# Horizon1026/Feature_Detector

Hardware: AMD Instinct MI355X
Metric: Mpix/s corner-response+NMS, 640x480 gray batch, 1/2/4/8 MI355X (higher is better)
Workload: dtype u8->i32/f32; 1 GPU; harris response+NMS + grid NMS (greedy min-distance select), 640x480 gray, batch 1/GPU (BASELINE configs[1]); detector=harris, rows=480, cols=640, global_batch=1, need=200, min_feature_distance=20, parallelism=frame-sharded x1 (no collective), graph=True

## Files before the change

### feature_detector_amd/csrc/fd_device.h

```cpp
#pragma once

#include <hip/hip_runtime.h>
#include <stdint.h>

namespace fdk {

constexpr int kWave = 64;

__device__ __forceinline__ int lane_id() { return threadIdx.x & 63; }

__device__ __forceinline__ uint32_t from_left(uint32_t v) {
    return static_cast<uint32_t>(__builtin_amdgcn_mov_dpp(static_cast<int>(v), 0x138, 0xF, 0xF, true));
}
__device__ __forceinline__ uint32_t from_right(uint32_t v) {
    return static_cast<uint32_t>(__builtin_amdgcn_mov_dpp(static_cast<int>(v), 0x130, 0xF, 0xF, true));
}
__device__ __forceinline__ float from_left_f(float v) { return __uint_as_float(from_left(__float_as_uint(v))); }
__device__ __forceinline__ float from_right_f(float v) { return __uint_as_float(from_right(__float_as_uint(v))); }

__device__ __forceinline__ __amdgpu_buffer_rsrc_t make_rsrc(const void *base, uint32_t bytes) {
    return __builtin_amdgcn_make_buffer_rsrc(const_cast<void *>(base), 0, static_cast<int>(bytes), 0x00020000);
}
__device__ __forceinline__ uint32_t buf_load_u32(__amdgpu_buffer_rsrc_t r, int32_t byte_off) {
    return static_cast<uint32_t>(__builtin_amdgcn_raw_buffer_load_b32(r, byte_off, 0, 0));
}
__device__ __forceinline__ uint32_t buf_load_u8(__amdgpu_buffer_rsrc_t r, int32_t byte_off) {
    return static_cast<uint32_t>(__builtin_amdgcn_raw_buffer_load_b8(r, byte_off, 0, 0));
}

__device__ __forceinline__ int win_byte(uint32_t L, uint32_t M, uint32_t R, int j) {
    const uint32_t w = j < 0 ? L : (j < 4 ? M : R);
    const int sh = 8 * (j < 0 ? j + 4 : (j < 4 ? j : j - 4));
    return static_cast<int>((w >> sh) & 0xFFu);
}

__device__ __forceinline__ float max3f(float a, float b, float c) {
    float r;
    asm("v_max3_f32 %0, %1, %2, %3" : "=v"(r) : "v"(a), "v"(b), "v"(c));
    return r;
}

__device__ __forceinline__ uint32_t add3u(uint32_t a, uint32_t b, uint32_t c) {
    uint32_t r;
    asm("v_add3_u32 %0, %1, %2, %3" : "=v"(r) : "v"(a), "v"(b), "v"(c));
    return r;
}

__device__ __forceinline__ uint32_t wave_incl_add(uint32_t x) {
    x += static_cast<uint32_t>(__builtin_amdgcn_update_dpp(0, static_cast<int>(x), 0x111, 0xF, 0xF, false));
    x += static_cast<uint32_t>(__builtin_amdgcn_update_dpp(0, static_cast<int>(x), 0x112, 0xF, 0xF, false));
    x += static_cast<uint32_t>(__builtin_amdgcn_update_dpp(0, static_cast<int>(x), 0x114, 0xF, 0xF, false));
    x += static_cast<uint32_t>(__builtin_amdgcn_update_dpp(0, static_cast<int>(x), 0x118, 0xF, 0xF, false));
    x += static_cast<uint32_t>(__builtin_amdgcn_update_dpp(0, static_cast<int>(x), 0x142, 0xA, 0xF, false));
    x += static_cast<uint32_t>(__builtin_amdgcn_update_dpp(0, static_cast<int>(x), 0x143, 0xC, 0xF, false));
    return x;
}
__device__ __forceinline__ uint32_t wave_max_u32(uint32_t x) {
    x = max(x, static_cast<uint32_t>(__builtin_amdgcn_update_dpp(0, static_cast<int>(x), 0x111, 0xF, 0xF, false)));
    x = max(x, static_cast<uint32_t>(__builtin_amdgcn_update_dpp(0, static_cast<int>(x), 0x112, 0xF, 0xF, false)));
    x = max(x, static_cast<uint32_t>(__builtin_amdgcn_update_dpp(0, static_cast<int>(x), 0x114, 0xF, 0xF, false)));
    x = max(x, static_cast<uint32_t>(__builtin_amdgcn_update_dpp(0, static_cast<int>(x), 0x118, 0xF, 0xF, false)));
    x = max(x, static_cast<uint32_t>(__builtin_amdgcn_update_dpp(0, static_cast<int>(x), 0x142, 0xA, 0xF, false)));
    x = max(x, static_cast<uint32_t>(__builtin_amdgcn_update_dpp(0, static_cast<int>(x), 0x143, 0xC, 0xF, false)));
    return static_cast<uint32_t>(__builtin_amdgcn_readlane(static_cast<int>(x), 63));
}
__device__ __forceinline__ uint32_t wave_min_u32(uint32_t x) {
    x = min(x, static_cast<uint32_t>(__builtin_amdgcn_update_dpp(-1, static_cast<int>(x), 0x111, 0xF, 0xF, false)));
    x = min(x, static_cast<uint32_t>(__builtin_amdgcn_update_dpp(-1, static_cast<int>(x), 0x112, 0xF, 0xF, false)));
    x = min(x, static_cast<uint32_t>(__builtin_amdgcn_update_dpp(-1, static_cast<int>(x), 0x114, 0xF, 0xF, false)));
    x = min(x, static_cast<uint32_t>(__builtin_amdgcn_update_dpp(-1, static_cast<int>(x), 0x118, 0xF, 0xF, false)));
    x = min(x, static_cast<uint32_t>(__builtin_amdgcn_update_dpp(-1, static_cast<int>(x), 0x142, 0xA, 0xF, false)));
    x = min(x, static_cast<uint32_t>(__builtin_amdgcn_update_dpp(-1, static_cast<int>(x), 0x143, 0xC, 0xF, false)));
    return static_cast<uint32_t>(__builtin_amdgcn_readlane(static_cast<int>(x), 63));
}
__device__ __forceinline__ uint32_t wave_total_add(uint32_t x) {
    return static_cast<uint32_t>(__builtin_amdgcn_readlane(static_cast<int>(wave_incl_add(x)), 63));
}
__device__ __forceinline__ uint32_t wave_suffix_add(uint32_t x) {
    const uint32_t p = wave_incl_add(x);
    const uint32_t tot = static_cast<uint32_t>(__builtin_amdgcn_readlane(static_cast<int>(p), 63));
    return tot - p + x;
}

__device__ __forceinline__ int opaque(int x) {
    asm volatile("" : "+v"(x));
    return x;
}

template <class T>
using lds_t = __attribute__((address_space(3))) T;
template <class T>
__device__ __forceinline__ lds_t<T> *to_lds(T *p) { return (lds_t<T> *)(p); }
template <class T>
__device__ __forceinline__ T *from_lds(lds_t<T> *p) { return (T *)(p); }

__device__ __forceinline__ uint64_t ballot(bool p) { return __ballot(p); }
__device__ __forceinline__ int popc64(uint64_t m) { return __popcll(m); }
__device__ __forceinline__ uint64_t lanes_below() {
    const int l = lane_id();
    return l == 0 ? 0ull : (~0ull >> (64 - l));
}

__device__ __forceinline__ int mbcnt64(uint64_t m, int acc) {
    const uint32_t lo = __builtin_amdgcn_mbcnt_lo(static_cast<uint32_t>(m), static_cast<uint32_t>(acc));
    return static_cast<int>(__builtin_amdgcn_mbcnt_hi(static_cast<uint32_t>(m >> 32), lo));
}

template <int NT>
__device__ __forceinline__ uint32_t wg_excl_add(uint32_t v, uint32_t *wsum, uint32_t &tot) {
    constexpr int kWaves = NT / kWave;
    const int lane = lane_id(), w = threadIdx.x / kWave;
    const uint32_t incl = wave_incl_add(v);
    if (lane == kWave - 1) wsum[w] = incl;
    __syncthreads();
    const uint32_t ws = lane < kWaves ? wsum[lane] : 0u;
    const uint32_t wincl = wave_incl_add(ws);
    const uint32_t wbase = static_cast<uint32_t>(__shfl(static_cast<int>(wincl - ws), w));
    tot = static_cast<uint32_t>(__builtin_amdgcn_readlane(static_cast<int>(wincl), kWaves - 1));
    __syncthreads();
    return wbase + incl - v;
}

__device__ __forceinline__ uint32_t float_key(float f) {
    const uint32_t u = __float_as_uint(f);
    return (u & 0x80000000u) ? ~u : (u | 0x80000000u);
}

typedef float f2 __attribute__((ext_vector_type(2)));

__device__ __forceinline__ f2 sqrt_rn_rsq2(f2 x) {
    const f2 xt = x + 0x1p-110f;
    const f2 y = {__builtin_amdgcn_rsqf(xt.x), __builtin_amdgcn_rsqf(xt.y)};
    const f2 s0 = x * y;
    const f2 e = __builtin_elementwise_fma(-s0, s0, x);
    const f2 h = y * 0.5f;
    return __builtin_elementwise_fma(e, h, s0);
}

}
```

### feature_detector_amd/csrc/fd_emit.h

```cpp
#pragma once

#include "fd_device.h"
#include "fd_kernels.h"

namespace fdk {

__device__ __forceinline__ uint32_t sel_key32(float resp, uint32_t key_base, int key_lz) {
    return (float_key(resp) - key_base) << key_lz;
}
__device__ __forceinline__ uint64_t sel_key64(float resp, uint32_t idx, uint32_t key_base, int key_lz, int tie_desc) {
    return (static_cast<uint64_t>(sel_key32(resp, key_base, key_lz)) << 32) | static_cast<uint64_t>(tie_desc ? idx : ~idx);
}
__device__ __forceinline__ uint32_t level0_bin(float resp, uint32_t key_base, int key_lz) {
    return sel_key32(resp, key_base, key_lz) >> 20;
}
__device__ __forceinline__ uint32_t level0_floor_key(uint32_t bin, uint32_t key_base, int key_lz) {
    return key_base + ((bin << 20) >> key_lz);
}

struct ListFrame {
    float *resp;
    uint32_t *idx;
    int64_t cap;
};
__device__ __forceinline__ ListFrame list_frame(const CandList &l, int f) {
    return {l.resp + static_cast<int64_t>(f) * l.cap, l.idx + static_cast<int64_t>(f) * l.cap, l.cap};
}

constexpr int kPixWg = 256;
constexpr int kHistPer = kHistBins / (4 * kPixWg);
__device__ __forceinline__ void hist_clear(uint32_t *h) {
    uint4 *h4 = reinterpret_cast<uint4 *>(h);
#pragma unroll
    for (int k = 0; k < kHistPer; ++k) h4[threadIdx.x + k * kPixWg] = make_uint4(0u, 0u, 0u, 0u);
    __syncthreads();
}
__device__ __forceinline__ void hist_flush(const uint32_t *h, uint32_t *g) {
    __syncthreads();
    constexpr int kPer = kHistBins / kPixWg;
    uint32_t v[kPer];
#pragma unroll
    for (int k = 0; k < kPer; ++k) v[k] = h[threadIdx.x + k * kPixWg];
#pragma unroll
    for (int k = 0; k < kPer; ++k)
        if (v[k]) atomicAdd(&g[threadIdx.x + k * kPixWg], v[k]);
}

__device__ __forceinline__ void wave_append(const CandList &l, int f, const float *sr, const uint32_t *si, int n,
                                            uint32_t *hist) {
    uint32_t base = 0;
    if (lane_id() == 0) base = atomicAdd(&l.count[f], static_cast<uint32_t>(n));
    base = __builtin_amdgcn_readfirstlane(base);
    const ListFrame d = list_frame(l, f);
    for (int i = lane_id(); i < n; i += kWave) {
        const float r = sr[i];
        if (hist) atomicAdd(&hist[level0_bin(r, l.key_base, l.key_lz)], 1u);
        const int64_t pos = static_cast<int64_t>(base) + i;
        if (pos < d.cap) {
            d.resp[pos] = r;
            d.idx[pos] = si[i];
        }
    }
}

template <class Src>
__device__ __forceinline__ void seg_list_flush(Src &src, const PointsArgs &a, int f, int g, bool active, uint32_t *hist,
                                               const uint32_t *ovf, uint32_t (&wtot)[4], uint32_t &wg_base) {
    const int tid = threadIdx.x, lane = lane_id(), wv = tid >> 6;
    if (!active) src.n = 0;
    const uint32_t wn = src.wave_total();
    if (lane == 0) wtot[wv] = wn;
    __syncthreads();
    if (*ovf) {
        if (active) src.flush(a, f);
        hist_flush(hist, a.list.hist0 + static_cast<int64_t>(f) * kHistBins);
        return;
    }
    uint32_t seg_base_early = 0;
    const uint32_t seg_total = wtot[0] + wtot[1] + wtot[2] + wtot[3];
    if (tid == 0 && seg_total) seg_base_early = atomicAdd(&a.list.count[f], seg_total);
    const uint32_t kb = a.list.key_base;
    const int lz = a.list.key_lz;
    if (!src.counted()) src.visit([&](float r, uint32_t) { atomicAdd(&hist[level0_bin(r, kb, lz)], 1u); });
    hist_flush(hist, a.list.hist0 + static_cast<int64_t>(f) * kHistBins);
    __syncthreads();
    constexpr int kPer = kHistBins / kPixWg;
    uint32_t v[kPer], sum = 0;
#pragma unroll
    for (int k = 0; k < kPer; ++k) sum += (v[k] = hist[kHistBins - 1 - (tid * kPer + k)]);
    const uint32_t incl = wave_incl_add(sum);
    if (lane == kWave - 1) wtot[wv] = incl;
    __syncthreads();
    uint32_t run = incl - sum, total = 0;
    for (int q = 0; q < 4; ++q) {
        run += q < wv ? wtot[q] : 0u;
        total += wtot[q];
    }
#pragma unroll
    for (int k = 0; k < kPer; ++k) {
        hist[kHistBins - 1 - (tid * kPer + k)] = run;
        run += v[k];
    }
    const int64_t seg = static_cast<int64_t>(f) * a.blocks_per_frame + g;
    if (tid == 0) {
        wg_base = seg_base_early;
        a.segdesc[seg] = make_uint2(wg_base, total);
    }
    __syncthreads();
    const ListFrame d = list_frame(a.list, f);
    const int64_t base = wg_base;
    uint64_t *head = a.seghead + seg * kSegHead;
    src.visit([&](float r, uint32_t id) {
        const uint32_t lp = atomicAdd(&hist[level0_bin(r, kb, lz)], 1u);
        const int64_t pos = base + lp;
        if (pos < d.cap) {
            d.resp[pos] = r;
            d.idx[pos] = id;
        }
        if (lp < static_cast<uint32_t>(kSegHead)) head[lp] = sel_key64(r, id, kb, lz, 0);
    });
    src.n = 0;
}

}
```

### feature_detector_amd/csrc/fd_points.hip

```cpp
#include "fd_corner_common.h"

namespace fdk {

namespace {

constexpr int kStage = FD_STAGE_CORNER;
constexpr int kStageFast = FD_STAGE_FAST;

struct Sink {
    float *resp;
    uint32_t *idx;
    uint32_t *hist;
    int n;
    uint32_t *ovf;
    uint32_t *ehist = nullptr;
    int cap = kStage;
};

__device__ __forceinline__ void sink_flush(Sink &sk, const PointsArgs &a, int f) {
    if (sk.n == 0) return;
    __builtin_amdgcn_fence(__ATOMIC_RELEASE, "wavefront");
    __builtin_amdgcn_wave_barrier();
    __builtin_amdgcn_fence(__ATOMIC_ACQUIRE, "wavefront");
    wave_append(a.list, f, sk.resp, sk.idx, sk.n, sk.hist);
    __builtin_amdgcn_fence(__ATOMIC_RELEASE, "wavefront");
    __builtin_amdgcn_wave_barrier();
    __builtin_amdgcn_fence(__ATOMIC_ACQUIRE, "wavefront");
    __builtin_amdgcn_s_waitcnt(0x0F70);
    sk.n = 0;
}

struct SinkSource {
    Sink &sk;
    int &n = sk.n;
    __device__ __forceinline__ uint32_t wave_total() const { return static_cast<uint32_t>(n); }
    __device__ __forceinline__ bool counted() const { return sk.ehist != nullptr; }
    template <class F>
    __device__ __forceinline__ void visit(F &&fn) const {
        for (int i = lane_id(); i < n; i += kWave) fn(sk.resp[i], sk.idx[i]);
    }
    __device__ __forceinline__ void flush(const PointsArgs &a, int f) { sink_flush(sk, a, f); }
};

template <bool RASTER, int SEGCAP>
__device__ __forceinline__ void emit_row(Sink &sk, const PointsArgs &a, int f, int tx, int row, int c0,
                                         const uint64_t (&b)[4], const bool (&fl)[4], const float (&v)[4]) {
    const uint64_t b0 = b[0], b1 = b[1], b2 = b[2], b3 = b[3];
    const int tot = popc64(b0) + popc64(b1) + popc64(b2) + popc64(b3);
    const uint32_t id0 = static_cast<uint32_t>(row) * static_cast<uint32_t>(a.cols) + static_cast<uint32_t>(c0);
    if constexpr (RASTER) {
        int pos = mbcnt64(b3, mbcnt64(b2, mbcnt64(b1, mbcnt64(b0, 0))));
        const int64_t seg = (static_cast<int64_t>(f) * a.rows + row) * a.tiles_x + tx;
        if (lane_id() == 0) a.seg_cnt[seg] = tot;
        Cand *dst = a.seg + seg * SEGCAP;
#pragma unroll
        for (int m = 0; m < 4; ++m)
            if (fl[m]) dst[pos++] = Cand{v[m], id0 + m};
    } else {
        if (tot == 0) return;
        if (sk.n + tot > sk.cap) {
            if (a.segdesc && lane_id() == 0) {
                atomicOr(&a.seg_bad[f], 1u);
                *sk.ovf = 1u;
            }
            sink_flush(sk, a, f);
        }
        int pos = mbcnt64(b3, mbcnt64(b2, mbcnt64(b1, mbcnt64(b0, sk.n))));
#pragma unroll
        for (int m = 0; m < 4; ++m)
            if (fl[m]) {
                if (sk.ehist) atomicAdd(&sk.ehist[level0_bin(v[m], a.list.key_base, a.list.key_lz)], 1u);
                sk.resp[pos] = v[m];
                sk.idx[pos] = id0 + m;
                ++pos;
            }
        sk.n += tot;
    }
}

__device__ __forceinline__ uint32_t mask_bits4(const PointsArgs &a, int f, int row, int c0) {
    if (c0 < 0 || c0 >= a.cols) return 0u;
    const uint32_t w = a.mask[(static_cast<int64_t>(f) * a.rows + row) * a.mask_wpr + (c0 >> 5)];
    return (w >> (c0 & 31)) & 0xFu;
}

template <int S>
struct alignas(16) DetectLdsT {
    float resp[4][S];
    uint32_t idx[4][S];
    uint32_t hist[kHistBins];
};
using DetectLds = DetectLdsT<kStage>;
static_assert(sizeof(DetectLds) % 16 == 0 && offsetof(DetectLds, hist) % 16 == 0, "uint4 histogram access");

template <int KIND, bool RASTER, bool MASKED, bool ALIGNED, bool G1>
__device__ __forceinline__ void corner_tile(const PointsArgs &a, int f, int ty, int tx, Sink &sk);

template <int KIND, bool RASTER, bool MASKED, bool ALIGNED, bool G1>
__global__ __launch_bounds__(256) void k_corner(PointsArgs a) {
    __shared__ DetectLds lds_all[1];
    int f, ty, tx;
    const bool active = decode_tile(a, f, ty, tx);
    __shared__ uint32_t seg_ovf;
    Sink sk{nullptr, nullptr, nullptr, 0, &seg_ovf};
    if constexpr (!RASTER) {
        const int wv = threadIdx.x >> 6;
        sk = Sink{lds_all[0].resp[wv], lds_all[0].idx[wv], a.list.hist0 ? lds_all[0].hist : nullptr, 0, &seg_ovf};
        if (threadIdx.x == 0) seg_ovf = 0;
        if (a.list.hist0) hist_clear(lds_all[0].hist);
        else __syncthreads();
    }
    if (active) corner_tile<KIND, RASTER, MASKED, ALIGNED, G1>(a, f, ty, tx, sk);
    if constexpr (!RASTER) {
        if (a.segdesc) {
            __shared__ uint32_t seg_wtot[4], seg_base;
            SinkSource src{sk};
            seg_list_flush(src, a, f, logical_block() % a.blocks_per_frame, active, lds_all[0].hist, &seg_ovf, seg_wtot, seg_base);
        } else {
            if (active) sink_flush(sk, a, f);
            if (a.list.hist0) hist_flush(lds_all[0].hist, a.list.hist0 + static_cast<int64_t>(f) * kHistBins);
        }
    }
}

template <int KIND, bool RASTER, bool MASKED, bool ALIGNED, bool G1>
__device__ __forceinline__ void corner_tile(const PointsArgs &a, int f, int ty, int tx, Sink &sk) {
    const int lane = lane_id();
    const int rows = a.rows, cols = a.cols;
    const int c0 = tx * kTileW + 4 * (lane - 1);
    const int y0 = 2 + ty * a.tile_h;
    const int y1 = min(y0 + a.tile_h, rows - 2);
    const auto rs = make_rsrc(a.frames + static_cast<int64_t>(f) * rows * cols, static_cast<uint32_t>(rows * cols));
    const bool tile_interior = tx * kTileW - 4 >= 2 && tx * kTileW + 4 * 62 + 3 <= cols - 3;

    bool cval[4], colv[4];
    uint64_t colv_b[4];
#pragma unroll
    for (int m = 0; m < 4; ++m) {
        cval[m] = c0 + m >= 2 && c0 + m <= cols - 3;
        colv[m] = cval[m] && lane >= 1 && lane <= 62;
        colv_b[m] = ballot(colv[m]);
    }

    uint32_t hxx[3][4], hyy[3][4], hxy[3][4];
    float rsp[3][4];
#pragma unroll
    for (int s = 0; s < 3; ++s)
#pragma unroll
        for (int m = 0; m < 4; ++m) hxx[s][m] = hyy[s][m] = hxy[s][m] = 0, rsp[s][m] = 0.0f;

    const int n_in = (y1 - y0) + 6;
    uint32_t ring[6];
#pragma unroll
    for (int t = 0; t < 6; ++t) ring[t] = t < 3 ? load_px4<ALIGNED>(rs, (y0 - 3 + t) * cols + c0) : 0u;
    __builtin_amdgcn_s_waitcnt(0x0F70);
    for (int i0 = 0; i0 < n_in; i0 += 6) {
#pragma unroll
        for (int t = 0; t < 6; ++t) {
            if (i0 + t >= n_in) break;
            const int s = t % 3, su = (t + 1) % 3, sc = (t + 2) % 3;
            const int ri = y0 - 3 + i0 + t;
            ring[(t + 3) % 6] = load_px4<ALIGNED>(rs, (ri + 3) * cols + c0);
            const uint32_t P_s = ring[t], P_su = ring[(t + 4) % 6], P_sc = ring[(t + 5) % 6];
            if (!(t >= 2 || i0 > 0)) continue;

            const uint32_t Lc = from_left(P_sc), Rc = from_right(P_sc);
            uint32_t qxx[6], qyy[6], qxy[6];
            uint32_t bsq = kBiasSq, bxy = kBiasXy;
            asm volatile("" : "+s"(bsq), "+s"(bxy));
#pragma unroll
            for (int m = 0; m < 4; ++m) {
                const int ix = win_byte(Lc, P_sc, Rc, m + 1) - win_byte(Lc, P_sc, Rc, m - 1);
                const int iy = win_byte(0, P_s, 0, m) - win_byte(0, P_su, 0, m);
                qxx[m + 1] = static_cast<uint32_t>(ix * ix) + bsq;
                qyy[m + 1] = static_cast<uint32_t>(iy * iy) + bsq;
                qxy[m + 1] = static_cast<uint32_t>(ix * iy) + bxy;
            }
            qxx[0] = from_left(qxx[4]);
            qyy[0] = from_left(qyy[4]);
            qxy[0] = from_left(qxy[4]);
            qxx[5] = from_right(qxx[1]);
            qyy[5] = from_right(qyy[1]);
            qxy[5] = from_right(qxy[1]);
#pragma unroll
            for (int m = 0; m < 4; ++m) {
                hxx[sc][m] = add3u(qxx[m], qxx[m + 1], qxx[m + 2]);
                hyy[sc][m] = add3u(qyy[m], qyy[m + 1], qyy[m + 2]);
                hxy[sc][m] = add3u(qxy[m], qxy[m + 1], qxy[m + 2]);
            }

            if (!(t >= 4 || i0 > 0)) continue;
            const int rr = ri - 2;
            const bool rowv = rr >= 2 && rr <= rows - 3;
            uint32_t sxx[4], syy[4], sxy[4];
#pragma unroll
            for (int m = 0; m < 4; ++m) {
                sxx[m] = add3u(hxx[s][m], hxx[su][m], hxx[sc][m]);
                syy[m] = add3u(hyy[s][m], hyy[su][m], hyy[sc][m]);
                sxy[m] = add3u(hxy[s][m], hxy[su][m], hxy[sc][m]);
            }
            const f2 r01 = corner_response2<KIND, G1>(sxx[0], sxx[1], syy[0], syy[1], sxy[0], sxy[1], a.thr);
            const f2 r23 = corner_response2<KIND, G1>(sxx[2], sxx[3], syy[2], syy[3], sxy[2], sxy[3], a.thr);
            const float r[4] = {r01.x, r01.y, r23.x, r23.y};
            if (!MASKED && rowv && tile_interior) {
#pragma unroll
                for (int m = 0; m < 4; ++m) rsp[su][m] = r[m];
            } else {
                uint32_t mb = 0xFu;
                if constexpr (MASKED) mb = rowv ? mask_bits4(a, f, rr, c0) : 0u;
#pragma unroll
                for (int m = 0; m < 4; ++m) rsp[su][m] = (rowv && cval[m] && ((mb >> m) & 1u)) ? r[m] : 0.0f;
            }

            const int nr = ri - 3;
            if (nr >= y0 && nr < y1) {
                const float lft = from_left_f(rsp[s][3]);
                const float rgt = from_right_f(rsp[s][0]);
                bool fl[4];
                float v[4];
                uint64_t b[4];
#pragma unroll
                for (int m = 0; m < 4; ++m) {
                    const float x = rsp[s][m];
                    const float xl = m == 0 ? lft : rsp[s][m - 1];
                    const float xr = m == 3 ? rgt : rsp[s][m + 1];
                    const float nb = max3f(max3f(xl, xr, a.thr), rsp[sc][m], rsp[su][m]);
                    const bool hit = x > nb;
                    v[m] = x;
                    fl[m] = colv[m] && hit;
                    b[m] = ballot(hit) & colv_b[m];
                }
                emit_row<RASTER, kSegCorner>(sk, a, f, tx, nr, c0, b, fl, v);
                if constexpr (RASTER) {
                    if (a.resp_map != nullptr) {
                        float *mrow = a.resp_map + (static_cast<int64_t>(f) * rows + nr) * cols;
#pragma unroll
                        for (int m = 0; m < 4; ++m)
                            if (colv[m]) mrow[c0 + m] = v[m];
                    }
                }
            }
        }
    }
}

constexpr uint32_t kH = 0x80808080u;
constexpr uint32_t kL = 0x7F7F7F7Fu;
constexpr uint32_t kOnes = 0x01010101u;

__device__ __forceinline__ uint32_t swar_gt(uint32_t x, uint32_t y, uint32_t yk) {
    const uint32_t z = (x | kH) - yk;
    return (x & ~y) | (~(x ^ y) & z);
}
__device__ __forceinline__ uint32_t swar_adds15(uint32_t p) {
    const uint32_t t = (p & kL) + 0x0F0F0F0Fu;
    const uint32_t ov = p & t & kH;
    const uint32_t ovm = (ov - (ov >> 7)) | ov;
    return t | (p & kH) | ovm;
}
__device__ __forceinline__ uint32_t swar_subs15(uint32_t p) {
    const uint32_t d = (p | kH) - 0x0F0F0F0Fu;
    const uint32_t un = ~p & ~d & kH;
    const uint32_t unm = (un - (un >> 7)) | un;
    return (d ^ (~p & kH)) & ~unm;
}
template <int DX>
__device__ __forceinline__ uint32_t shifted(uint32_t L, uint32_t P, uint32_t R) {
    if constexpr (DX == 0) return P;
    else if constexpr (DX > 0) return __builtin_amdgcn_alignbyte(R, P, DX);
    else return __builtin_amdgcn_alignbyte(P, L, 4 + DX);
}

__device__ __forceinline__ float fast_offset(int nseg, const int32_t *ks, const float *os, const float *inc, int32_t k) {
    int lo = 0, hi = nseg - 1;
    while (lo < hi) {
        const int mid = (lo + hi + 1) >> 1;
        if (ks[mid] <= k) lo = mid; else hi = mid - 1;
    }
    return __builtin_fmaf(static_cast<float>(k - ks[lo]), inc[lo], os[lo]);
}

template <bool RASTER, bool MASKED, bool ALIGNED>
__device__ __forceinline__ void fast_tile(const PointsArgs &a, const FastOffsets &off, const int32_t *seg_k,
                                          const float *seg_o, const float *seg_inc, int f, int ty, int tx, Sink &sk,
                                          float cut, uint32_t &skip);

template <bool RASTER, bool MASKED, bool ALIGNED>
__global__ __launch_bounds__(256) void k_fast(PointsArgs a, FastOffsets off) {
    __shared__ DetectLdsT<kStageFast> lds_all[1];
    __shared__ int32_t seg_k[kMaxOffsetSegs];
    __shared__ float seg_o[kMaxOffsetSegs], seg_inc[kMaxOffsetSegs];
    __shared__ uint32_t seg_ovf;
    __shared__ uint32_t seg_wtot[4], seg_base;
    int f, ty, tx;
    const bool active = decode_tile(a, f, ty, tx);
    if (a.emit_cut_next && blockIdx.x == 0 && threadIdx.x == 0) *a.emit_cut_next = 0x7F800000u;
    const float cut = a.emit_cut ? __uint_as_float(*a.emit_cut) : -__builtin_inff();
    for (int i = threadIdx.x; i < off.nseg; i += blockDim.x) {
        seg_k[i] = static_cast<int32_t>(off.k_start[i]);
        seg_o[i] = static_cast<float>(off.o_start[i]);
        seg_inc[i] = static_cast<float>(off.inc[i]);
    }
    auto run = [&](int fr) {
        uint32_t skip = 0;
        Sink sk{nullptr, nullptr, nullptr, 0, &seg_ovf};
        if constexpr (!RASTER) {
            const int wv = threadIdx.x >> 6;
            sk = Sink{lds_all[0].resp[wv], lds_all[0].idx[wv], a.list.hist0 ? lds_all[0].hist : nullptr, 0, &seg_ovf};
            sk.ehist = sk.hist;
            sk.hist = nullptr;
            sk.cap = kStageFast;
            if (threadIdx.x == 0) seg_ovf = 0;
            if (a.list.hist0) hist_clear(lds_all[0].hist);
            else __syncthreads();
        } else {
            __syncthreads();
        }
        if (active) fast_tile<RASTER, MASKED, ALIGNED>(a, off, seg_k, seg_o, seg_inc, fr, ty, tx, sk, cut, skip);
        if (a.skipped && skip && lane_id() == 0) atomicAdd(&a.skipped[fr], skip);
        if constexpr (!RASTER) {
            if (a.segdesc) {
                SinkSource src{sk};
                seg_list_flush(src, a, fr, logical_block() % a.blocks_per_frame, active, lds_all[0].hist, &seg_ovf, seg_wtot, seg_base);
            } else {
                if (active) sink_flush(sk, a, fr);
                if (a.list.hist0) hist_flush(lds_all[0].hist, a.list.hist0 + static_cast<int64_t>(fr) * kHistBins);
            }
        }
    };
    if (a.redo_status) {
        for (int base = 0; base < a.batch; base += kWave) {
            const int fr = base + lane_id();
            uint64_t m = ballot(fr < a.batch && (a.redo_status[min(fr, a.batch - 1)] & kFrameRedo));
            while (m) {
                const int j = __builtin_ctzll(m);
                m &= m - 1ull;
                __syncthreads();
                run(base + j);
            }
        }
        return;
    }
    run(f);
}

template <bool RASTER, bool MASKED, bool ALIGNED>
__device__ __forceinline__ void fast_tile(const PointsArgs &a, const FastOffsets &off, const int32_t *seg_k,
                                          const float *seg_o, const float *seg_inc, int f, int ty, int tx, Sink &sk,
                                          float cut, uint32_t &skip) {
    const int lane = lane_id();
    const int rows = a.rows, cols = a.cols;
    const int c0 = tx * kTileW + 4 * (lane - 1);
    const int y0 = 3 + ty * a.tile_h;
    const int y1 = min(y0 + a.tile_h, rows - 3);
    const auto rs = make_rsrc(a.frames + static_cast<int64_t>(f) * rows * cols, static_cast<uint32_t>(rows * cols));
    const auto lut = make_rsrc(off.run_lut, 65536u);

    bool colv[4];
    uint32_t colmask = 0;
#pragma unroll
    for (int m = 0; m < 4; ++m) {
        colv[m] = lane >= 1 && lane <= 62 && c0 + m >= 3 && c0 + m <= cols - 4;
        colmask |= colv[m] ? (0x80u << (8 * m)) : 0u;
    }
    const int cmin = max(tx * kTileW, 3), cmax = min(tx * kTileW + kTileW - 1, cols - 4);
    int sg = 0;

    uint32_t P[7], L[7], R[7];
#pragma unroll
    for (int s = 0; s < 7; ++s) P[s] = L[s] = R[s] = 0;

    auto finish_row = [&](int orow, uint32_t live, const int (&score)[4]) {
        float resp[4];
        bool fl[4];
        if constexpr (MASKED) {
            int32_t kbase = 0;
            uint32_t mword = 0;
            const int64_t rb = static_cast<int64_t>(f) * rows + orow;
            kbase = a.row_base[rb];
            if (c0 >= 0 && c0 < cols) {
                const int w = c0 >> 5;
                kbase += a.word_pref[rb * a.mask_wpr + w];
                mword = a.mask[rb * a.mask_wpr + w];
                if (w == 0) mword &= ~7u;
            }
#pragma unroll
            for (int m = 0; m < 4; ++m) {
                const bool lv = (live >> (8 * m + 7)) & 1u;
                const int32_t k = kbase + __popc(mword & ((1u << ((c0 + m) & 31)) - 1u));
                resp[m] = 0.0f;
                if (lv && (score[m] > 0 || k >= off.k0))
                    resp[m] = static_cast<float>(score[m]) + fast_offset(off.nseg, seg_k, seg_o, seg_inc, k);
                fl[m] = lv && resp[m] > a.thr;
            }
        } else {
            const int32_t krow = (orow - 3) * (cols - 6) - 3;
            const int32_t kmin = krow + cmin, kmax = krow + cmax;
            while (sg + 1 < off.nseg && seg_k[sg + 1] <= kmin) ++sg;
            if (sg + 1 >= off.nseg || seg_k[sg + 1] > kmax) {
                const float os = seg_o[sg], inc = seg_inc[sg];
                const int32_t kr = krow + c0 - seg_k[sg];
#pragma unroll
                for (int m = 0; m < 4; ++m) {
                    resp[m] = static_cast<float>(score[m]) + __builtin_fmaf(static_cast<float>(kr + m), inc, os);
                    fl[m] = colv[m] && resp[m] > a.thr;
                }
            } else {
#pragma unroll
                for (int m = 0; m < 4; ++m) {
                    resp[m] = 0.0f;
                    if (colv[m]) resp[m] = static_cast<float>(score[m]) +
                                           fast_offset(off.nseg, seg_k, seg_o, seg_inc, krow + c0 + m);
                    fl[m] = colv[m] && resp[m] > a.thr;
                }
            }
        }
        if constexpr (!RASTER) {
            bool em[4];
#pragma unroll
            for (int m = 0; m < 4; ++m) {
                em[m] = fl[m] && resp[m] >= cut;
                skip += static_cast<uint32_t>(popc64(ballot(fl[m] && !em[m])));
                fl[m] = em[m];
            }
        }
        const uint64_t b[4] = {ballot(fl[0]), ballot(fl[1]), ballot(fl[2]), ballot(fl[3])};
        emit_row<RASTER, kSegFast>(sk, a, f, tx, orow, c0, b, fl, resp);
        if constexpr (RASTER) {
            if (a.resp_map != nullptr) {
                float *mrow = a.resp_map + (static_cast<int64_t>(f) * rows + orow) * cols;
#pragma unroll
                for (int m = 0; m < 4; ++m)
                    if (fl[m]) mrow[c0 + m] = resp[m];
            }
        }
    };
    bool pend = false;
    int p_orow = 0;
    uint32_t p_live = 0, p_pass = 0;
    uint32_t p_sb[4] = {0u, 0u, 0u, 0u}, p_sd[4] = {0u, 0u, 0u, 0u};
    auto finish_pending = [&]() {
        int score[4];
#pragma unroll
        for (int m = 0; m < 4; ++m) score[m] = ((p_pass >> (8 * m + 7)) & 1u) ? static_cast<int>(max(p_sb[m], p_sd[m])) : 0;
        finish_row(p_orow, p_live, score);
    };

    const int n_in = (y1 - y0) + 6;
    uint32_t nxt = load_px4<ALIGNED>(rs, (y0 - 3) * cols + c0);
    for (int i0 = 0; i0 < n_in; i0 += 7) {
#pragma unroll
        for (int s = 0; s < 7; ++s) {
            const int ri = y0 - 3 + i0 + s;
            P[s] = nxt;
            nxt = load_px4<ALIGNED>(rs, (ri + 1) * cols + c0);
            L[s] = from_left(P[s]);
            R[s] = from_right(P[s]);
            const int orow = ri - 3;
            if (orow < y0 || orow >= y1) continue;
#define ROW(dy) L[(s + 4 + (dy)) % 7], P[(s + 4 + (dy)) % 7], R[(s + 4 + (dy)) % 7]
            const uint32_t p = P[(s + 4) % 7];
            const uint32_t tb = swar_adds15(p), td = swar_subs15(p);
            const uint32_t tbk = (tb & kL) + kOnes;
            const uint32_t tdk = (td | kH) - kOnes;
            auto bright = [&](uint32_t v) { return swar_gt(v, tb, tbk); };
            auto dark = [&](uint32_t v) {
                const uint32_t z = tdk - (v & kL);
                return (td & ~v) | (~(td ^ v) & z);
            };
            uint32_t live = colmask;
            if constexpr (MASKED) {
                const uint32_t mb = mask_bits4(a, f, orow, c0);
                live &= ((mb & 1u) ? 0x80u : 0u) | ((mb & 2u) ? 0x8000u : 0u) | ((mb & 4u) ? 0x800000u : 0u) |
                        ((mb & 8u) ? 0x80000000u : 0u);
            }
            const uint32_t v4 = shifted<3>(ROW(0)), v8 = P[(s + 7) % 7], v12 = shifted<-3>(ROW(0));
            const uint32_t b4 = bright(v4), b8 = bright(v8), b12 = bright(v12);
            const uint32_t d4 = dark(v4), d8 = dark(v8), d12 = dark(v12);
            const uint32_t pass = ((b4 & b8 & b12) | (d4 & d8 & d12)) & live;
            uint32_t sb[4] = {0u, 0u, 0u, 0u}, sd[4] = {0u, 0u, 0u, 0u};
            if (ballot(pass != 0u) != 0ull) {
                uint32_t blo, bhi, dlo, dhi;
                auto put = [](uint32_t &acc, uint32_t g) { acc = (g & kH) | ((acc >> 1) & kL); };
                const uint32_t v0 = shifted<0>(ROW(-3)), v1 = shifted<1>(ROW(-3)), v2 = shifted<2>(ROW(-2));
                const uint32_t v3 = shifted<3>(ROW(-1)), v5 = shifted<3>(ROW(1)), v6 = shifted<2>(ROW(2));
                const uint32_t v7 = shifted<1>(ROW(3));
                blo = bright(v0); dlo = dark(v0);
                put(blo, bright(v1)); put(dlo, dark(v1));
                put(blo, bright(v2)); put(dlo, dark(v2));
                put(blo, bright(v3)); put(dlo, dark(v3));
                put(blo, b4); put(dlo, d4);
                put(blo, bright(v5)); put(dlo, dark(v5));
                put(blo, bright(v6)); put(dlo, dark(v6));
                put(blo, bright(v7)); put(dlo, dark(v7));
                const uint32_t v9 = shifted<-1>(ROW(3)), v10 = shifted<-2>(ROW(2)), v11 = shifted<-3>(ROW(1));
                const uint32_t v13 = shifted<-3>(ROW(-1)), v14 = shifted<-2>(ROW(-2)), v15 = shifted<-1>(ROW(-3));
                bhi = b8; dhi = d8;
                put(bhi, bright(v9)); put(dhi, dark(v9));
                put(bhi, bright(v10)); put(dhi, dark(v10));
                put(bhi, bright(v11)); put(dhi, dark(v11));
                put(bhi, b12); put(dhi, d12);
                put(bhi, bright(v13)); put(dhi, dark(v13));
                put(bhi, bright(v14)); put(dhi, dark(v14));
                put(bhi, bright(v15)); put(dhi, dark(v15));
#pragma unroll
                for (int m = 0; m < 4; ++m) {
                    if ((pass >> (8 * m + 7)) & 1u) {
                        const uint32_t sel = 0x0C0C0000u | (static_cast<uint32_t>(4 + m) << 8) | static_cast<uint32_t>(m);
                        const uint32_t ib = __builtin_amdgcn_perm(bhi, blo, sel);
                        const uint32_t id = __builtin_amdgcn_perm(dhi, dlo, sel);
                        sb[m] = buf_load_u8(lut, static_cast<int32_t>(ib));
                        sd[m] = buf_load_u8(lut, static_cast<int32_t>(id));
                    }
                }
            }
#undef ROW
            if (pend) finish_pending();
            pend = true;
            p_orow = orow;
            p_live = live;
            p_pass = pass;
#pragma unroll
            for (int m = 0; m < 4; ++m) {
                p_sb[m] = sb[m];
                p_sd[m] = sd[m];
            }
        }
    }
    if (pend) finish_pending();
}

__global__ __launch_bounds__(256) void k_mask_boxes(const float *prior_xy, const int32_t *prior_frame, int n_prior,
                                                    int dist, int rows, int cols, uint32_t *mask, int wpr) {
    const int span = 2 * dist + 1;
    const int64_t t = static_cast<int64_t>(blockIdx.x) * blockDim.x + threadIdx.x;
    if (t >= static_cast<int64_t>(n_prior) * span) return;
    const int p = static_cast<int>(t / span);
    const int dr = static_cast<int>(t % span) - dist;
    const int r0 = static_cast<int>(prior_xy[2 * p + 1]);
    const int cc = static_cast<int>(prior_xy[2 * p + 0]);
    const int r = r0 + dr;
    if (r < 0 || r > rows - 1) return;
    const int ca = max(cc - dist, 0), cb = min(cc + dist, cols - 1);
    if (ca > cb) return;
    uint32_t *row = mask + (static_cast<int64_t>(prior_frame[p]) * rows + r) * wpr;
    for (int w = ca >> 5; w <= (cb >> 5); ++w) {
        const int lo = max(ca - 32 * w, 0), hi = min(cb - 32 * w, 31);
        const uint32_t bits = (hi == 31 ? 0xFFFFFFFFu : ((1u << (hi + 1)) - 1u)) & ~((1u << lo) - 1u);
        atomicAnd(&row[w], ~bits);
    }
}

__global__ __launch_bounds__(1024) void k_fast_mask_scan(const uint32_t *mask, int wpr, int rows, int cols,
                                                         int32_t *row_base, int32_t *word_pref) {
    __shared__ int32_t tot[4096];
    const int f = blockIdx.x;
    const uint32_t *fm = mask + static_cast<int64_t>(f) * rows * wpr;
    for (int r = threadIdx.x; r < rows; r += blockDim.x) {
        int acc = 0;
        const bool rv = r >= 3 && r <= rows - 4;
        for (int w = 0; w < wpr; ++w) {
            word_pref[(static_cast<int64_t>(f) * rows + r) * wpr + w] = acc;
            uint32_t bits = rv ? fm[static_cast<int64_t>(r) * wpr + w] : 0u;
            const int lo = 3 - 32 * w, hi = (cols - 4) - 32 * w;
            if (hi < 0) bits = 0;
            else if (hi < 31) bits &= (1u << (hi + 1)) - 1u;
            if (lo > 31) bits = 0;
            else if (lo > 0) bits &= ~((1u << lo) - 1u);
            acc += __popc(bits);
        }
        if (r < 4096) tot[r] = acc;
    }
    __syncthreads();
    if (threadIdx.x == 0) {
        int64_t acc = 0;
        for (int r = 0; r < rows; ++r) {
            row_base[static_cast<int64_t>(f) * rows + r] = static_cast<int32_t>(acc);
            acc += tot[r];
        }
    }
}

__global__ __launch_bounds__(1024) void k_compact(CompactArgs a) {
    __shared__ int64_t wsum[16];
    __shared__ int64_t carry;
    const int f = blockIdx.x;
    const int tid = threadIdx.x, lane = lane_id(), wv = tid >> 6;
    const int nseg = (a.row_hi - a.row_lo) * a.tiles_x;
    const int32_t *cnt = a.seg_cnt + (static_cast<int64_t>(f) * a.rows + a.row_lo) * a.tiles_x;
    const Cand *seg = a.seg + (static_cast<int64_t>(f) * a.rows + a.row_lo) * a.tiles_x * a.seg_cap;
    float *oresp = a.out_resp + static_cast<int64_t>(f) * a.cap;
    int32_t *ox = a.out_x + static_cast<int64_t>(f) * a.cap;
    int32_t *oy = a.out_y + static_cast<int64_t>(f) * a.cap;
    if (tid == 0) carry = 0;
    __syncthreads();
    for (int s0 = 0; s0 < nseg; s0 += 1024) {
        const int s = s0 + tid;
        const int c = s < nseg ? cnt[s] : 0;
        int64_t incl = c;
        for (int o = 1; o < kWave; o <<= 1) {
            const int64_t t = __shfl_up(incl, o);
            if (lane >= o) incl += t;
        }
        if (lane == 63) wsum[wv] = incl;
        __syncthreads();
        int64_t wpre = 0;
        for (int q = 0; q < wv; ++q) wpre += wsum[q];
        const int64_t start = carry + wpre + incl - c;
        __syncthreads();
        if (tid == 1023) carry = start + c;
        for (int e = 0; e < c; ++e) {
            const int64_t pos = start + e;
            if (pos < a.cap) {
                const Cand cd = seg[static_cast<int64_t>(s) * a.seg_cap + e];
                const int y = static_cast<int>(cd.idx / static_cast<uint32_t>(a.cols));
                oresp[pos] = cd.resp;
                ox[pos] = static_cast<int32_t>(cd.idx - static_cast<uint32_t>(y) * a.cols);
                oy[pos] = y;
            }
        }
        __syncthreads();
    }
    if (tid == 0) a.out_counts[f] = carry;
}

}

static inline int blocks_for_waves(const PointsArgs &a) {
    return a.batch * a.blocks_per_frame;
}

hipError_t launch_corner(int kind, bool raster, const PointsArgs &a, hipStream_t s) {
    const dim3 grid(blocks_for_waves(a)), block(256);
    if (!raster && a.px != 0) return launch_corner_lp_any(kind, a, s);
    const bool masked = a.mask != nullptr, aligned = a.aligned4 != 0;
    const bool g1 = !raster && a.thr >= 0.0f;
#define FD_CORNER_A(K, RS, M, G)                                                                \
    do {                                                                                        \
        if (aligned) hipLaunchKernelGGL((k_corner<K, RS, M, true, G>), grid, block, 0, s, a);  \
        else hipLaunchKernelGGL((k_corner<K, RS, M, false, G>), grid, block, 0, s, a);         \
    } while (0)
#define FD_CORNER(K, RS, M)                                      \
    do {                                                         \
        if (RS) FD_CORNER_A(K, RS, M, false);                    \
        else if (g1) FD_CORNER_A(K, false, M, true);             \
        else FD_CORNER_A(K, false, M, false);                    \
    } while (0)
    if (kind == 0) {
        if (raster) { if (masked) FD_CORNER(0, true, true); else FD_CORNER(0, true, false); }
        else { if (masked) FD_CORNER(0, false, true); else FD_CORNER(0, false, false); }
    } else {
        if (raster) { if (masked) FD_CORNER(1, true, true); else FD_CORNER(1, true, false); }
        else { if (masked) FD_CORNER(1, false, true); else FD_CORNER(1, false, false); }
    }
#undef FD_CORNER
#undef FD_CORNER_A
    return hipGetLastError();
}

hipError_t launch_fast(bool raster, const PointsArgs &a, const FastOffsets &off, hipStream_t s) {
    const dim3 grid(a.redo_status ? a.blocks_per_frame : blocks_for_waves(a)), block(256);
    const bool masked = a.mask != nullptr, aligned = a.aligned4 != 0;
#define FD_FAST(RS, M)                                                                          \
    do {                                                                                        \
        if (aligned) hipLaunchKernelGGL((k_fast<RS, M, true>), grid, block, 0, s, a, off);     \
        else hipLaunchKernelGGL((k_fast<RS, M, false>), grid, block, 0, s, a, off);            \
    } while (0)
    if (raster) { if (masked) FD_FAST(true, true); else FD_FAST(true, false); }
    else { if (masked) FD_FAST(false, true); else FD_FAST(false, false); }
#undef FD_FAST
    return hipGetLastError();
}

hipError_t launch_mask_boxes(const float *prior_xy, const int32_t *prior_frame, int n_prior, int dist, int rows,
                             int cols, uint32_t *mask, int mask_wpr, hipStream_t s) {
    if (n_prior <= 0 || dist < 0) return hipSuccess;
    const int64_t threads = static_cast<int64_t>(n_prior) * (2 * dist + 1);
    hipLaunchKernelGGL(k_mask_boxes, dim3(static_cast<unsigned>((threads + 255) / 256)), dim3(256), 0, s, prior_xy,
                       prior_frame, n_prior, dist, rows, cols, mask, mask_wpr);
    return hipGetLastError();
}

hipError_t launch_fast_mask_scan(const uint32_t *mask, int mask_wpr, int batch, int rows, int cols, int32_t *row_base,
                                 int32_t *word_pref, hipStream_t s) {
    hipLaunchKernelGGL(k_fast_mask_scan, dim3(batch), dim3(1024), 0, s, mask, mask_wpr, rows, cols, row_base,
                       word_pref);
    return hipGetLastError();
}

hipError_t launch_compact(const CompactArgs &a, int batch, hipStream_t s) {
    hipLaunchKernelGGL(k_compact, dim3(batch), dim3(1024), 0, s, a);
    return hipGetLastError();
}

}
```

Baseline: 12170 Mpix/s.

## Add short-tile corner kernel with two columns per lane and 512-thread workgroups

Adds a specialized corner-response+NMS kernel for 3-row tiles in which each lane handles two columns instead of four, using 16-bit loads and edge-lane halo loads. Workgroups grow to eight waves so more tiles run concurrently, which raises parallelism on a small 640x480 frame. The histogram and segment-flush helpers are templated on workgroup size to support this. It runs only when the host picks tile_h equal to 3 with segment descriptors, and it adds per-wave halo loads and more DPP exchanges per pixel.

```diff
diff --git a/feature_detector_amd/csrc/fd_device.h b/feature_detector_amd/csrc/fd_device.h
--- a/feature_detector_amd/csrc/fd_device.h
+++ b/feature_detector_amd/csrc/fd_device.h
@@ -23,6 +23,9 @@
 }
 __device__ __forceinline__ uint32_t buf_load_u32(__amdgpu_buffer_rsrc_t r, int32_t byte_off) {
     return static_cast<uint32_t>(__builtin_amdgcn_raw_buffer_load_b32(r, byte_off, 0, 0));
+}
+__device__ __forceinline__ uint32_t buf_load_u16(__amdgpu_buffer_rsrc_t r, int32_t byte_off) {
+    return static_cast<uint16_t>(__builtin_amdgcn_raw_buffer_load_b16(r, byte_off, 0, 0));
 }
 __device__ __forceinline__ uint32_t buf_load_u8(__amdgpu_buffer_rsrc_t r, int32_t byte_off) {
     return static_cast<uint32_t>(__builtin_amdgcn_raw_buffer_load_b8(r, byte_off, 0, 0));
diff --git a/feature_detector_amd/csrc/fd_emit.h b/feature_detector_amd/csrc/fd_emit.h
--- a/feature_detector_amd/csrc/fd_emit.h
+++ b/feature_detector_amd/csrc/fd_emit.h
@@ -28,22 +28,24 @@
 }
 
 constexpr int kPixWg = 256;
-constexpr int kHistPer = kHistBins / (4 * kPixWg);
+template <int WG = kPixWg>
 __device__ __forceinline__ void hist_clear(uint32_t *h) {
+    constexpr int kHistPer = kHistBins / (4 * WG);
     uint4 *h4 = reinterpret_cast<uint4 *>(h);
 #pragma unroll
-    for (int k = 0; k < kHistPer; ++k) h4[threadIdx.x + k * kPixWg] = make_uint4(0u, 0u, 0u, 0u);
+    for (int k = 0; k < kHistPer; ++k) h4[threadIdx.x + k * WG] = make_uint4(0u, 0u, 0u, 0u);
     __syncthreads();
 }
+template <int WG = kPixWg>
 __device__ __forceinline__ void hist_flush(const uint32_t *h, uint32_t *g) {
     __syncthreads();
-    constexpr int kPer = kHistBins / kPixWg;
+    constexpr int kPer = kHistBins / WG;
     uint32_t v[kPer];
 #pragma unroll
-    for (int k = 0; k < kPer; ++k) v[k] = h[threadIdx.x + k * kPixWg];
+    for (int k = 0; k < kPer; ++k) v[k] = h[threadIdx.x + k * WG];
 #pragma unroll
     for (int k = 0; k < kPer; ++k)
-        if (v[k]) atomicAdd(&g[threadIdx.x + k * kPixWg], v[k]);
+        if (v[k]) atomicAdd(&g[threadIdx.x + k * WG], v[k]);
 }
 
 __device__ __forceinline__ void wave_append(const CandList &l, int f, const float *sr, const uint32_t *si, int n,
@@ -63,9 +65,10 @@
     }
 }
 
-template <class Src>
+template <int WG = kPixWg, class Src>
 __device__ __forceinline__ void seg_list_flush(Src &src, const PointsArgs &a, int f, int g, bool active, uint32_t *hist,
-                                               const uint32_t *ovf, uint32_t (&wtot)[4], uint32_t &wg_base) {
+                                               const uint32_t *ovf, uint32_t (&wtot)[WG / kWave], uint32_t &wg_base) {
+    constexpr int kWaves = WG / kWave;
     const int tid = threadIdx.x, lane = lane_id(), wv = tid >> 6;
     if (!active) src.n = 0;
     const uint32_t wn = src.wave_total();
@@ -73,18 +76,20 @@
     __syncthreads();
     if (*ovf) {
         if (active) src.flush(a, f);
-        hist_flush(hist, a.list.hist0 + static_cast<int64_t>(f) * kHistBins);
+        hist_flush<WG>(hist, a.list.hist0 + static_cast<int64_t>(f) * kHistBins);
         return;
     }
     uint32_t seg_base_early = 0;
-    const uint32_t seg_total = wtot[0] + wtot[1] + wtot[2] + wtot[3];
+    uint32_t seg_total = wtot[0] + wtot[1] + wtot[2] + wtot[3];
+#pragma unroll
+    for (int q = 4; q < kWaves; ++q) seg_total += wtot[q];
     if (tid == 0 && seg_total) seg_base_early = atomicAdd(&a.list.count[f], seg_total);
     const uint32_t kb = a.list.key_base;
     const int lz = a.list.key_lz;
     if (!src.counted()) src.visit([&](float r, uint32_t) { atomicAdd(&hist[level0_bin(r, kb, lz)], 1u); });
-    hist_flush(hist, a.list.hist0 + static_cast<int64_t>(f) * kHistBins);
+    hist_flush<WG>(hist, a.list.hist0 + static_cast<int64_t>(f) * kHistBins);
     __syncthreads();
-    constexpr int kPer = kHistBins / kPixWg;
+    constexpr int kPer = kHistBins / WG;
     uint32_t v[kPer], sum = 0;
 #pragma unroll
     for (int k = 0; k < kPer; ++k) sum += (v[k] = hist[kHistBins - 1 - (tid * kPer + k)]);
@@ -92,7 +97,7 @@
     if (lane == kWave - 1) wtot[wv] = incl;
     __syncthreads();
     uint32_t run = incl - sum, total = 0;
-    for (int q = 0; q < 4; ++q) {
+    for (int q = 0; q < kWaves; ++q) {
         run += q < wv ? wtot[q] : 0u;
         total += wtot[q];
     }
diff --git a/feature_detector_amd/csrc/fd_points.hip b/feature_detector_amd/csrc/fd_points.hip
--- a/feature_detector_amd/csrc/fd_points.hip
+++ b/feature_detector_amd/csrc/fd_points.hip
@@ -83,11 +83,17 @@
     const uint32_t w = a.mask[(static_cast<int64_t>(f) * a.rows + row) * a.mask_wpr + (c0 >> 5)];
     return (w >> (c0 & 31)) & 0xFu;
 }
-
-template <int S>
+template <int NC>
+__device__ __forceinline__ uint32_t mask_bits(const PointsArgs &a, int f, int row, int c0) {
+    if (c0 < 0 || c0 >= a.cols) return 0u;
+    const uint32_t w = a.mask[(static_cast<int64_t>(f) * a.rows + row) * a.mask_wpr + (c0 >> 5)];
+    return (w >> (c0 & 31)) & ((1u << NC) - 1u);
+}
+
+template <int S, int W = 4>
 struct alignas(16) DetectLdsT {
-    float resp[4][S];
-    uint32_t idx[4][S];
+    float resp[W][S];
+    uint32_t idx[W][S];
     uint32_t hist[kHistBins];
 };
 using DetectLds = DetectLdsT<kStage>;
@@ -242,6 +248,207 @@
             }
         }
     }
+}
+
+constexpr int kShortTileH = 3;
+constexpr int kShortCols = 2;
+static_assert(kShortCols == 2 || kShortCols == 4, "columns per lane of the short-tile kernel");
+constexpr int kShortWg = kWave * 4 * (4 / kShortCols);
+constexpr int kShortStage = kShortCols == 2 ? 252 : kStage;
+static_assert(kShortStage >= 62 * kShortCols * kShortTileH / 2, "a short tile's candidates fit the staging");
+using ShortLds = DetectLdsT<kShortStage, kShortWg / kWave>;
+static_assert(sizeof(ShortLds) + 4 * (kShortWg / kWave + 2) <= 32768, "32 KiB of LDS per workgroup");
+static_assert(sizeof(ShortLds) % 16 == 0 && offsetof(ShortLds, hist) % 16 == 0, "uint4 histogram access");
+
+template <int NC, bool ALIGNED>
+__device__ __forceinline__ uint32_t load_pxn(__amdgpu_buffer_rsrc_t r, int32_t off) {
+    if constexpr (NC == 4) return load_px4<ALIGNED>(r, off);
+    else if constexpr (ALIGNED) return buf_load_u16(r, off);
+    else return buf_load_u8(r, off) | (buf_load_u8(r, off + 1) << 8);
+}
+template <int NC>
+__device__ __forceinline__ int px_byte(uint32_t L, uint32_t M, uint32_t R, int j) {
+    const uint32_t w = j < 0 ? L : (j < NC ? M : R);
+    const int sh = 8 * (j < 0 ? NC - 1 : (j < NC ? j : 0));
+    return static_cast<int>((w >> sh) & 0xFFu);
+}
+
+template <int NC>
+__device__ __forceinline__ void emit_short(Sink &sk, const PointsArgs &a, int f, int row, int c0,
+                                           const uint64_t (&b)[NC], const bool (&fl)[NC], const float (&v)[NC]) {
+    int tot = 0;
+#pragma unroll
+    for (int m = 0; m < NC; ++m) tot += popc64(b[m]);
+    if (tot == 0) return;
+    if (sk.n + tot > sk.cap) {
+        if (lane_id() == 0) {
+            atomicOr(&a.seg_bad[f], 1u);
+            *sk.ovf = 1u;
+        }
+        sink_flush(sk, a, f);
+    }
+    int pos = sk.n;
+#pragma unroll
+    for (int m = 0; m < NC; ++m) pos = mbcnt64(b[m], pos);
+    const uint32_t id0 = static_cast<uint32_t>(row) * static_cast<uint32_t>(a.cols) + static_cast<uint32_t>(c0);
+#pragma unroll
+    for (int m = 0; m < NC; ++m)
+        if (fl[m]) {
+            sk.resp[pos] = v[m];
+            sk.idx[pos] = id0 + m;
+            ++pos;
+        }
+    sk.n += tot;
+}
+
+template <int T>
+struct StepC {
+    static constexpr int value = T;
+};
+
+template <int KIND, bool MASKED, bool ALIGNED, int NC>
+__device__ __forceinline__ void corner_tile_short(const PointsArgs &a, int f, int ty, int tx, Sink &sk) {
+    constexpr int TW = 62 * NC;
+    constexpr int kRows = kShortTileH + 6;
+    const int lane = lane_id();
+    const int rows = a.rows, cols = a.cols;
+    const int c0 = tx * TW + NC * (lane - 1);
+    const int y0 = 2 + ty * kShortTileH;
+    const int y1 = min(y0 + kShortTileH, rows - 2);
+    const int n_in = (y1 - y0) + 6;
+    const auto rs = make_rsrc(a.frames + static_cast<int64_t>(f) * rows * cols, static_cast<uint32_t>(rows * cols));
+    uint32_t P[kRows];
+#pragma unroll
+    for (int t = 0; t < kRows; ++t) P[t] = load_pxn<NC, ALIGNED>(rs, (y0 - 3 + t) * cols + c0);
+    uint32_t E[kRows];
+#pragma unroll
+    for (int t = 0; t < kRows; ++t) E[t] = 0u;
+    if constexpr (NC == 2) {
+        if (lane == 0 || lane == 63) {
+            const int eoff = lane == 0 ? -NC : NC;
+#pragma unroll
+            for (int t = 0; t < kRows; ++t) E[t] = load_pxn<NC, ALIGNED>(rs, (y0 - 3 + t) * cols + c0 + eoff);
+        }
+    }
+
+    const bool tile_interior = tx * TW - NC >= 2 && tx * TW + NC * 62 + NC - 1 <= cols - 3;
+    bool cval[NC], colv[NC];
+    uint64_t colv_b[NC];
+#pragma unroll
+    for (int m = 0; m < NC; ++m) {
+        cval[m] = c0 + m >= 2 && c0 + m <= cols - 3;
+        colv[m] = cval[m] && lane >= 1 && lane <= 62;
+        colv_b[m] = ballot(colv[m]);
+    }
+
+    uint32_t hxx[kRows][NC], hyy[kRows][NC], hxy[kRows][NC];
+    float rsp[kRows][NC];
+    auto step = [&](auto tc) {
+        constexpr int t = decltype(tc)::value;
+        const uint32_t P_s = P[t], P_sc = P[t - 1], P_su = P[t - 2];
+        const uint32_t Lc = static_cast<uint32_t>(__builtin_amdgcn_update_dpp(static_cast<int>(E[t - 1]), static_cast<int>(P_sc), 0x138, 0xF, 0xF, false));
+        const uint32_t Rc = static_cast<uint32_t>(__builtin_amdgcn_update_dpp(static_cast<int>(E[t - 1]), static_cast<int>(P_sc), 0x130, 0xF, 0xF, false));
+        uint32_t qxx[NC + 2], qyy[NC + 2], qxy[NC + 2];
+        uint32_t bsq = kBiasSq, bxy = kBiasXy;
+        asm volatile("" : "+s"(bsq), "+s"(bxy));
+#pragma unroll
+        for (int m = 0; m < NC; ++m) {
+            const int ix = px_byte<NC>(Lc, P_sc, Rc, m + 1) - px_byte<NC>(Lc, P_sc, Rc, m - 1);
+            const int iy = px_byte<NC>(0, P_s, 0, m) - px_byte<NC>(0, P_su, 0, m);
+            qxx[m + 1] = static_cast<uint32_t>(ix * ix) + bsq;
+            qyy[m + 1] = static_cast<uint32_t>(iy * iy) + bsq;
+            qxy[m + 1] = static_cast<uint32_t>(ix * iy) + bxy;
+        }
+        qxx[0] = from_left(qxx[NC]);
+        qyy[0] = from_left(qyy[NC]);
+        qxy[0] = from_left(qxy[NC]);
+        qxx[NC + 1] = from_right(qxx[1]);
+        qyy[NC + 1] = from_right(qyy[1]);
+        qxy[NC + 1] = from_right(qxy[1]);
+#pragma unroll
+        for (int m = 0; m < NC; ++m) {
+            hxx[t][m] = add3u(qxx[m], qxx[m + 1], qxx[m + 2]);
+            hyy[t][m] = add3u(qyy[m], qyy[m + 1], qyy[m + 2]);
+            hxy[t][m] = add3u(qxy[m], qxy[m + 1], qxy[m + 2]);
+        }
+
+        if constexpr (t >= 4) {
+            const int rr = y0 - 5 + t;
+            const bool rowv = rr >= 2 && rr <= rows - 3;
+            float r[NC];
+#pragma unroll
+            for (int m = 0; m < NC; m += 2) {
+                uint32_t sxx[2], syy[2], sxy[2];
+#pragma unroll
+                for (int k = 0; k < 2; ++k) {
+                    sxx[k] = add3u(hxx[t][m + k], hxx[t - 2][m + k], hxx[t - 1][m + k]);
+                    syy[k] = add3u(hyy[t][m + k], hyy[t - 2][m + k], hyy[t - 1][m + k]);
+                    sxy[k] = add3u(hxy[t][m + k], hxy[t - 2][m + k], hxy[t - 1][m + k]);
+                }
+                const f2 rp = corner_response2<KIND, true>(sxx[0], sxx[1], syy[0], syy[1], sxy[0], sxy[1], a.thr);
+                r[m] = rp.x;
+                r[m + 1] = rp.y;
+            }
+            if (!MASKED && rowv && tile_interior) {
+#pragma unroll
+                for (int m = 0; m < NC; ++m) rsp[t][m] = r[m];
+            } else {
+                uint32_t mb = (1u << NC) - 1u;
+                if constexpr (MASKED) mb = rowv ? mask_bits<NC>(a, f, rr, c0) : 0u;
+#pragma unroll
+                for (int m = 0; m < NC; ++m) rsp[t][m] = (rowv && cval[m] && ((mb >> m) & 1u)) ? r[m] : 0.0f;
+            }
+
+            if constexpr (t >= 6) {
+                const int nr = y0 - 6 + t;
+                const float lft = from_left_f(rsp[t - 1][NC - 1]);
+                const float rgt = from_right_f(rsp[t - 1][0]);
+                bool fl[NC];
+                float v[NC];
+                uint64_t b[NC];
+#pragma unroll
+                for (int m = 0; m < NC; ++m) {
+                    const float x = rsp[t - 1][m];
+                    const float xl = m == 0 ? lft : rsp[t - 1][m - 1];
+                    const float xr = m == NC - 1 ? rgt : rsp[t - 1][m + 1];
+                    const float nb = max3f(max3f(xl, xr, a.thr), rsp[t][m], rsp[t - 2][m]);
+                    const bool hit = x > nb;
+                    v[m] = x;
+                    fl[m] = colv[m] && hit;
+                    b[m] = ballot(hit) & colv_b[m];
+                }
+                emit_short<NC>(sk, a, f, nr, c0, b, fl, v);
+            }
+        }
+    };
+    step(StepC<2>{});
+    step(StepC<3>{});
+    step(StepC<4>{});
+    step(StepC<5>{});
+    step(StepC<6>{});
+    if (n_in > 7) step(StepC<7>{});
+    if (n_in > 8) step(StepC<8>{});
+}
+
+template <int KIND, bool MASKED, bool ALIGNED>
+__global__ __launch_bounds__(kShortWg) void k_corner_short(PointsArgs a) {
+    constexpr int NC = kShortCols, W = kShortWg / kWave;
+    __shared__ ShortLds lds;
+    __shared__ uint32_t seg_ovf, seg_wtot[W], seg_base;
+    const int lb = logical_block();
+    const int f = lb / a.blocks_per_frame, g = lb % a.blocks_per_frame;
+    const int wv = threadIdx.x >> 6;
+    const int tiles_x = a.tiles_x * (4 / NC);
+    const int t = __builtin_amdgcn_readfirstlane(g * W + wv);
+    const int tx = t % tiles_x, ty = t / tiles_x;
+    const bool active = t < tiles_x * a.tiles_y;
+    Sink sk{lds.resp[wv], lds.idx[wv], lds.hist, 0, &seg_ovf};
+    sk.cap = kShortStage;
+    if (threadIdx.x == 0) seg_ovf = 0;
+    hist_clear<kShortWg>(lds.hist);
+    if (active) corner_tile_short<KIND, MASKED, ALIGNED, NC>(a, f, ty, tx, sk);
+    SinkSource src{sk};
+    seg_list_flush<kShortWg>(src, a, f, g, active, lds.hist, &seg_ovf, seg_wtot, seg_base);
 }
 
 constexpr uint32_t kH = 0x80808080u;
@@ -635,6 +842,20 @@
     if (!raster && a.px != 0) return launch_corner_lp_any(kind, a, s);
     const bool masked = a.mask != nullptr, aligned = a.aligned4 != 0;
     const bool g1 = !raster && a.thr >= 0.0f;
+    if (g1 && a.segdesc && a.tile_h == kShortTileH) {
+        const dim3 wg(kShortWg);
+#define FD_SHORT(K)                                                                                      \
+    do {                                                                                                 \
+        if (masked && aligned) hipLaunchKernelGGL((k_corner_short<K, true, true>), grid, wg, 0, s, a);   \
+        else if (masked) hipLaunchKernelGGL((k_corner_short<K, true, false>), grid, wg, 0, s, a);        \
+        else if (aligned) hipLaunchKernelGGL((k_corner_short<K, false, true>), grid, wg, 0, s, a);       \
+        else hipLaunchKernelGGL((k_corner_short<K, false, false>), grid, wg, 0, s, a);                   \
+    } while (0)
+        if (kind == 0) FD_SHORT(0);
+        else FD_SHORT(1);
+#undef FD_SHORT
+        return hipGetLastError();
+    }
 #define FD_CORNER_A(K, RS, M, G)                                                                \
     do {                                                                                        \
         if (aligned) hipLaunchKernelGGL((k_corner<K, RS, M, true, G>), grid, block, 0, s, a);  \
```

Measured after the change: 12830 Mpix/s (median of 6 runs). +5.4%, better.
